# orybkin/video-gcp

Measured on AMD Instinct MI355X. Metric: predicted frames/sec, 64x64x3 seq_len=80 gcp_tree (posterior forward + all loss terms, model(inputs) and model.loss() of train.py:157-159, batch-stat BatchNorm), higher is better.
Workload: dtype f32 (encoder / decoder convs and the tree GEMMs from 512 rows: split-f16 MFMA with f32 accumulate, f32-equivalent; everything else exact f32 MFMA)

## Files before the change

include/gcpx.h:

```cpp
#ifndef GCPX_H
#define GCPX_H

#include <stdint.h>

#ifdef __cplusplus
extern "C" {
#endif

#define GCPX_VERSION 1

typedef enum gcpx_status {
    GCPX_OK = 0,
    GCPX_ERR_INVALID_ARG = -1,
    GCPX_ERR_UNSUPPORTED = -2,
    GCPX_ERR_HIP = -3,
    GCPX_ERR_COMM = -4
} gcpx_status;

typedef enum gcpx_act { GCPX_ACT_NONE = 0, GCPX_ACT_LRELU = 1, GCPX_ACT_TANH = 2 } gcpx_act;

int gcpx_version(void);
const char* gcpx_last_error(void);
int gcpx_conv_grid(void);

// ... 26 lines not shown
    int32_t Cout;
    int32_t out_pitch;
    int32_t upsample;
    int32_t out_act;
    int32_t head_mode;
    const float* wpk;
    const float* bias;
    float* out;
    float* images;
    float* stats_partial;
    const int32_t* raw_row_map;
    const int32_t* src_row_map;
    const int32_t* src_row_frames;
    int32_t n_src_rows;
    int32_t w_split_log2;
    const void* wpk_split;
    const int32_t* w_split_log2_dev;
    int32_t split_layout;
    int32_t nll_rows;
    const float* nll_target;
    float* nll_partial;
    const float* nll_row_weight;
    float nll_scale;
    int32_t _pad3;
    float* images_rows;
    int64_t images_rows_dup;
    const float* bwd_r;
    const float *bwd_scale, *bwd_shift, *bwd_mean, *bwd_rstd;
    const float* addend;
    int32_t addend_frame_div;
    int32_t _pad4;
} gcpx_conv_args;

typedef enum gcpx_split_layout { GCPX_SPLIT_PLAIN = 0, GCPX_SPLIT_ROWFOLD = 1, GCPX_SPLIT_HEAD32 = 2 } gcpx_split_layout;

int gcpx_conv3x3(const gcpx_conv_args* a, void* stream);
int gcpx_conv3x3_grid(const gcpx_conv_args* a);
int gcpx_conv4x4s2(const gcpx_conv_args* a, void* stream);
int gcpx_conv4x4s2_grid(void);
int gcpx_conv4x4s2_image(const float* x, const float* wpk, const float* bias, float* out,
                         int32_t F, int32_t Hin, int32_t Win, int32_t Cout, int32_t out_act, void* stream);

int gcpx_bn_finalize(const float* partial, int32_t n_partial, int32_t pitch, int32_t C, double count,
                     const float* gamma, const float* beta, float eps, float* scale, float* shift,
                     float* running_mean, float* running_var, float momentum, float* mean_out, float* rstd_out,
                     void* stream);
int gcpx_randn(float* out, int64_t n, uint64_t* state, void* stream);
int gcpx_bn_fold(const float* running_mean, const float* running_var, const float* gamma, const float* beta,
                 float eps, int32_t C, float* scale, float* shift, void* stream);

typedef struct gcpx_row_src {
    const float* ptr;
    const int32_t* rowidx;
    const float* scale;
    const float* shiftv;
    int64_t sb, sr;
    int32_t width;
    int32_t shift;
    int32_t act;
    int32_t cmod;
} gcpx_row_src;

typedef enum gcpx_gemm_epi {
    GCPX_EPI_NONE = 0,
    GCPX_EPI_LRELU = 1,
    GCPX_EPI_LSTM = 2,
    GCPX_EPI_GAUSS_SAMPLE = 3
// ... 500 lines not shown
```

video-gcp_amd/csrc/conv3x3_split.hip:

```cpp
#include "common.h"
#include "split_mfma.h"

#include <cstdlib>
#include <type_traits>

namespace {

struct SplitUpCfg {
    static constexpr int RW = 18, RH = 6, LW = 10, LH = 4, CC = 16, KS = 5;
    static constexpr int RAW_BYTES = LH * LW * CC * 4;
    static constexpr int PLANE_BYTES = RH * RW * 32;
    static constexpr int WAVE_BYTES = RAW_BYTES + 2 * PLANE_BYTES;
    static constexpr int NS = (LH * LW * 4 + 63) / 64;
    static constexpr int W_CHUNK_BYTES = KS * 2 * 1024;
    static int lds_bytes(int nchunk) { return nchunk * W_CHUNK_BYTES + 8 * WAVE_BYTES + 8 * 2 * 16 * 4; }
};

__global__ void __launch_bounds__(512, 2) conv3x3_up16_split_kernel(const gcpx_conv_args a, const int items_per_wave,
                                                                    const int nitems) {
    using Cfg = SplitUpCfg;
    constexpr int RW = Cfg::RW, RH = Cfg::RH, LW = Cfg::LW, LH = Cfg::LH, CC = Cfg::CC, NS = Cfg::NS, KS = Cfg::KS;
    extern __shared__ float4 smem4[];
    const int nchunk = a.Cin / CC;
    const char* wl = reinterpret_cast<const char*>(smem4);
    const int tid = threadIdx.x, lane = tid & 63;
    const int wave = __builtin_amdgcn_readfirstlane(tid >> 6);
    char* wbuf = reinterpret_cast<char*>(smem4) + nchunk * Cfg::W_CHUNK_BYTES + wave * Cfg::WAVE_BYTES;
    float* raw = reinterpret_cast<float*>(wbuf);
    char* hi = wbuf + Cfg::RAW_BYTES;
    float* red = reinterpret_cast<float*>(reinterpret_cast<char*>(smem4) + nchunk * Cfg::W_CHUNK_BYTES + 8 * Cfg::WAVE_BYTES);
    const int j = lane & 15, q = lane >> 4;
    const int H = a.Hout, W = a.Wout, Hin = a.Hin, Win = a.Win;
    const int ncb = W / 16, nrq = H / 4;

    for (int i = tid; i < nchunk * Cfg::W_CHUNK_BYTES / 16; i += 512) smem4[i] = reinterpret_cast<const float4*>(a.wpk_split)[i];
    __syncthreads();

// ... 1088 lines not shown
#pragma unroll
    for (int s = 1; s < 64; s <<= 1) m = fmaxf(m, __shfl_xor(m, s));
    if ((tid & 63) == 0) red[tid >> 6] = m;
    __syncthreads();
    m = red[0];
#pragma unroll
    for (int w = 1; w < 16; ++w) m = fmaxf(m, red[w]);
    int e = m > 0.f ? 14 + 127 - (int)((__float_as_uint(m) >> 23) & 0xff) : 0;
    e = max(-20, min(100, e));
    if (tid == 0) *log2_out = e;
    const float sc = __uint_as_float((unsigned)(127 + e) << 23);
    for (int i = tid; i < n; i += 1024) {
        const int k = idx[i];
        const float v = (k >= 0 ? theta[k] : 0.f) * sc;
        const _Float16 h1 = (_Float16)v;
        const _Float16 h2 = (_Float16)(v - (float)h1);
        const int o = (i >> 9) * 1024 + (i & 511);
        out[o] = h1;
        out[o + 512] = h2;
    }
}
}

extern "C" int gcpx_split_pack(const float* theta, const int32_t* idx, int32_t n, void* out, int32_t* log2_out, void* stream_) {
    GCPX_CHECK_ARG(theta && idx && out && log2_out, "null pointer");
    GCPX_CHECK_ARG(n > 0 && n % 512 == 0, "n must be a positive multiple of 512");
    hipLaunchKernelGGL(split_pack_kernel, dim3(1), dim3(1024), 0, reinterpret_cast<hipStream_t>(stream_), theta, idx, n,
                       reinterpret_cast<_Float16*>(out), log2_out);
    GCPX_CHECK_LAUNCH();
    return GCPX_OK;
}

int gcpx_launch_up32_split(const gcpx_conv_args* a, hipStream_t stream, int which, int grid) {
    if (which == 0) return launch_up32_split<2, 1>(a, stream, grid);
    if (which == 1) return launch_up32_split<2, 2>(a, stream, grid);
    return launch_up32_split<4, 2>(a, stream, grid);
}

int gcpx_launch_up16_fold(const gcpx_conv_args* a, hipStream_t stream, int grid) {
    using Cfg = FoldCfg;
    GCPX_CHECK_ARG(a->Cin == 32 && a->Cout == 16 && a->Hin % Cfg::R == 0 && a->Hout == 2 * a->Hin && a->Wout == 2 * a->Win && a->Wout % 16 == 0,
                   "row-folded block: 32 -> 16 channels, Hin a multiple of 4, output width a multiple of 16");
    GCPX_CHECK_ARG(a->src[0].C % 4 == 0 && (a->nsrc == 1 ? a->src[0].C == 32 : a->src[0].C + a->src[1].C == 32), "source channels");
    static const bool prio = getenv("GCPX_FOLD_NOPRIO") == nullptr;
    auto kern = prio ? conv3x3_up16_fold_kernel<true> : conv3x3_up16_fold_kernel<false>;
    static bool attr_set = false;
    if (!attr_set) {
        for (auto k : {conv3x3_up16_fold_kernel<true>, conv3x3_up16_fold_kernel<false>}) {
            hipError_t e = hipFuncSetAttribute(reinterpret_cast<const void*>(k), hipFuncAttributeMaxDynamicSharedMemorySize, Cfg::LDS_BYTES);
            if (e != hipSuccess) {
                gcpx_set_error("conv3x3 row-folded up16: hipFuncSetAttribute(%d B LDS): %s", Cfg::LDS_BYTES, hipGetErrorString(e));
                return GCPX_ERR_HIP;
            }
        }
        attr_set = true;
    }
    const int nitems = a->F * (a->Hin / Cfg::R) * (a->Wout / 16);
    const int ipw = (nitems + grid * 8 - 1) / (grid * 8);
    hipLaunchKernelGGL(kern, dim3(grid), dim3(512), Cfg::LDS_BYTES, stream, *a, ipw, nitems);
    GCPX_CHECK_LAUNCH();
    return GCPX_OK;
}

extern "C" int gcpx_fold_upsample_weights(const float* w, int32_t Cout, int32_t Cin, float* out, void* stream_) {
    GCPX_CHECK_ARG(w && out && Cout > 0 && Cin > 0, "bad arguments");
    const int n = 24 * Cout * Cin;
// ... 19 lines not shown
```

video-gcp_amd/forward_plan.py:

```python
import ctypes as C
import os
from contextlib import contextmanager

import torch

from . import packing as pk
from . import runtime as rt
from .hparams import GCPHParams
from .params import init_params, encoder_layers, encoder_skip_layers, decoder_layers
from .plan_ops import _Plan, _addr, N_LANES


class ForwardPlanMixin:

    def _plan_encoder(self, plan, tag, x_ptr, F, out_ptr, out_ob, out_orow, out_rpb):
        hp, P, lib = self._hp, self.pk, self.lib
        G = lib.gcpx_conv4x4s2_grid()
        S = hp.img_sz
        skip_idx = encoder_skip_layers(hp)
        skips = {}
        a0 = self._buf(f"{tag}.a0", (F, S // 2, S // 2, hp.ngf))
        enc_rec = dict(F=F, x_ptr=x_ptr, a0=a0, r={}, out=(out_ptr, out_ob, out_orow, out_rpb))
        plan.rec[f"enc:{tag}"] = enc_rec
        plan.add(f"enc.input:{tag}", lib.gcpx_conv4x4s2_image, x_ptr, P["enc.input.w"].data_ptr(),
# ... 37 lines not shown
        nrb = lib.gcpx_gemm_row_blocks(B * T, hp.nz_mid)
        st = self._buf(f"{tag}.st", (nrb, 2, hp.nz_mid)) if self.training else None
        self._gemm(plan, f"{tag}.pyramid-0", taps(y1, hp.nz_mid), B * T, hp.nz_mid, T, P[f"{tag}.pyramid-0.w"],
                   P[f"{tag}.pyramid-0.b"], out=y2.data_ptr(), ob=T * hp.nz_mid, orow=hp.nz_mid, stats=st)
        sc, sh = self._bn(plan, f"{tag}.bn", f"{prefix}.net.pyramid-0.norm", hp.nz_mid, st, nrb, hp.nz_mid, B * T)
        self._gemm(plan, f"{tag}.head", taps(y2, hp.nz_mid, scale=sc, shiftv=sh, act=rt.ACT_LRELU, cmod=hp.nz_mid),
                   B * T, nz, T, P[f"{tag}.head.w"], P[f"{tag}.head.b"], out=out.data_ptr(), ob=T * nz, orow=nz)

    def _plan_attention(self, plan, l, W, el, er, M, n, B, Kp, Vp, tin):
        hp, lib = self._hp, self.lib
        T, nz, dk = hp.max_seq_len, hp.nz_enc, hp.nz_attn_key
        li = l if hp.untied_layers else 0
        qin = self._buf(f"attn.qin{l}", (M, dk))
        self._mlp(plan, f"attn.query{l}", W["attn.query"], [el, er], M, n, out=qin.data_ptr(), ob=n * dk, orow=dk)
        dense = lambda t, w: self._rowsrc(t.data_ptr(), 0, w, w)
        qp = self._buf(f"attn.q{l}", (M, dk))
        self._gemm(plan, f"attn.q_proj{l}", [dense(qin, dk)], M, dk, M, W["attn.q_proj.w"], W["attn.q_proj.b"],
                   out=qp.data_ptr(), ob=0, orow=dk)
        o = self._buf(f"attn.o{l}", (M, nz))
        gamma = self._buf(f"attn.gamma{l}", (M, T))
        temp = self.sd[f"tree_module.tree_modules.{li}.inference.attention.attention_layers.0.temperature"]
        plan.add(f"attn{l}", lib.gcpx_attention, qp.data_ptr(), _addr(Kp, li * B * T * dk), _addr(Vp, li * B * T * nz), None,
                 tin["end_ind"].data_ptr(), temp.data_ptr(), o.data_ptr(), gamma.data_ptr(), M, n, T, dk, nz, hp.n_attention_heads)
        raw = self._buf(f"attn.raw{l}", (M, nz))
        self._gemm(plan, f"attn.out_proj{l}", [dense(o, nz)], M, nz, M, W["attn.out_proj.w"], W["attn.out_proj.b"],
                   out=raw.data_ptr(), ob=0, orow=nz)
        et = self._buf(f"attn.e_tilde{l}", (M, nz))
        self._gemm(plan, f"attn.out{l}", [dense(raw, nz)], M, nz, M, W["attn.out.w"], W["attn.out.b"], out=et.data_ptr(), ob=0, orow=nz)
        plan.rec.setdefault("gamma", {})[l] = gamma
        plan.rec.setdefault("e_tilde", {})[l] = et
        plan.rec.setdefault("attn", {})[l] = dict(qin=qin, qp=qp, o=o, raw=raw, gamma=gamma, et=et, M=M, n=n, li=li, temp=temp)
        return self._rowsrc(et.data_ptr(), n * nz, nz, nz)

    def _plan_decoder_features(self, plan, e_src, F, rpb, skips):
        hp, P, lib = self._hp, self.pk, self.lib
        ctop = self._c_top
        d0 = self._buf("dec.d0", (F, 4, 4, ctop))
        plan.rec["dec"] = dict(F=F, rpb=rpb, e_src=e_src, d0=d0, blocks=[], skips=skips)
        nrb = lib.gcpx_gemm_row_blocks(F, 16 * ctop)
        st = self._buf("dec.st0", (nrb, 2, 16 * ctop)) if self.training else None
        self._gemm(plan, "dec.input", [e_src], F, 16 * ctop, rpb, P["dec.input.w"], P["dec.input.b"], out=d0.data_ptr(),
                   ob=rpb * 16 * ctop, orow=16 * ctop, stats=st)
        sc, sh = self._bn(plan, "dec.bn0", "decoder.net.input.norm", ctop, st, nrb, 16 * ctop, F * 16)
        prev = (d0.data_ptr(), ctop, 1, sc, sh, rt.ACT_LRELU)
        res = 4
        for name, c_prev, c_skip, skip_idx, cout in decoder_layers(hp):
            srcs = [prev]
            if skip_idx >= 0:
                t, C_, ssc, ssh, sact = skips[skip_idx]
                assert C_ == c_skip and t.shape[1] == res
                srcs.append((t.data_ptr(), C_, rpb, ssc, ssh, sact))
            o = self._buf(f"dec.{name}", (F, 2 * res, 2 * res, cout))
            cpad = (cout + 15) // 16 * 16
            hoist = (skip_idx >= 0 and rpb > 1 and F % rpb == 0 and self.split_f16 and cout in (32, 64) and c_prev % 32 == 0 and
                     c_skip % 32 == 0 and f"dec.{name}" in self.pk_split and "fold" not in self.pk_split[f"dec.{name}"] and
                     os.environ.get("GCPX_NO_SKIP_HOIST") is None)
            addend = None
            if hoist:
                addend = self._buf(f"dec.{name}.skip", (F // rpb, 2 * res, 2 * res, cout))
                t, C_, ssc, ssh, sact = skips[skip_idx]
                zb = self._buf(f"dec.{name}.zero_bias", (cpad,), zero=True)
                a_s = self._conv_args([(t.data_ptr(), C_, 1, ssc, ssh, sact)], F // rpb, res, res, 2 * res, 2 * res, cout, cout,
                                      P[f"dec.{name}.w"], zb, addend, upsample=1)
                self._set_split(a_s, f"dec.{name}")
                a_s.wpk_split = a_s.wpk_split + (c_prev // 32) * 9 * (cpad // 16) * 2048
                plan.keep.append(a_s)
                plan.add(f"dec.{name}.skip", lib.gcpx_conv3x3, C.byref(a_s))
                srcs_main = [prev]
            else:
                srcs_main = srcs
            a = self._conv_args(srcs_main, F, res, res, 2 * res, 2 * res, cout, cout, P[f"dec.{name}.w"], P[f"dec.{name}.b"],
                                o, upsample=1, stats=(o if self.training else None))
            if hoist:
                a.addend, a.addend_frame_div = addend.data_ptr(), rpb
            self._set_split(a, f"dec.{name}")
            Gl = lib.gcpx_conv3x3_grid(C.byref(a))
            assert Gl > 0, rt.lib().gcpx_last_error()
            st = self._buf(f"dec.st.{name}", (Gl, 2, cpad)) if self.training else None
            a.stats_partial = st.data_ptr() if st is not None else None
            plan.keep.append(a)
            plan.add(f"dec.{name}", lib.gcpx_conv3x3, C.byref(a))
            plan.rec["dec"]["blocks"].append(dict(name=name, srcs=srcs, out=o, res_in=res, cout=cout, c_prev=c_prev, c_skip=c_skip,
                                                  skip_idx=skip_idx))
            res *= 2
            sc, sh = self._bn(plan, f"dec.bn.{name}", f"decoder.net.{name}.norm", cout, st, Gl, cpad, F * res * res)
            prev = (o.data_ptr(), cout, 1, sc, sh, rt.ACT_LRELU)
        assert res == hp.img_sz
        return prev

    def _build_plan(self, key, tin):
        hp, P, lib = self._hp, self.pk, self.lib
        B, has_traj, has_z, sample_prior, phase = key[0], key[1], key[2], key[3], key[4]
        pred_len = key[9]
        train_aux = has_traj and phase == "train" and not sample_prior
        L, T, N = hp.hierarchy_levels, hp.max_seq_len, hp.n_nodes
        nz, nv, H, SD = hp.nz_enc, hp.nz_vae, hp.nz_mid_lstm, hp.lstm_state_dim
        PS = 2 ** L + 1
        plan = _Plan(lib)
        G = lib.gcpx_conv_grid()
        def plan_aux_indices():
# ... 44 lines not shown
                if hp.seq_enc == "none":
                    inf_enc = enc_traj
                else:
                    inf_enc = self._buf("inf_enc_seq", (B * T, nz))
                    self._plan_seq_encoder(plan, "seq", "inf_encoder", enc_traj, inf_enc, B)
                if attentive:
                    dk = hp.nz_attn_key
                    n_mod = L if hp.untied_layers else 1
                    if hp.seq_enc == "none":
                        kenc = enc_traj
                    else:
                        kenc = self._buf("inf_key_enc", (B * T, nz))
                        self._plan_seq_encoder(plan, "kseq", "inf_key_encoder.0", enc_traj, kenc, B)
                    keys = self._buf("inf_enc_key_seq", (B * T, dk))
                    dense = lambda t, w: self._rowsrc(t.data_ptr(), 0, w, w)
                    self._gemm(plan, "kseq.key", [dense(kenc, nz)], B * T, dk, B * T, P["kseq.key.w"], P["kseq.key.b"],
                               out=keys.data_ptr(), ob=0, orow=dk)
                    Kp = self._buf("attn.K", (n_mod, B * T, dk))
                    Vp = self._buf("attn.V", (n_mod, B * T, nz))
                    self._gemm(plan, "attn.k_proj", [dense(keys, dk)], B * T, dk, B * T, P["attn.k_proj.w"], P["attn.k_proj.b"],
                               out=Kp.data_ptr(), ob=0, orow=dk, batch=(n_mod, 0, P["attn.k_proj.w"][0].numel(), dk, B * T * dk))
                    self._gemm(plan, "attn.v_proj", [dense(inf_enc, nz)], B * T, nz, B * T, P["attn.v_proj.w"], P["attn.v_proj.b"],
                               out=Vp.data_ptr(), ob=0, orow=nz, batch=(n_mod, 0, P["attn.v_proj.w"][0].numel(), nz, B * T * nz))
                    plan.rec["attn_kv"] = dict(Kp=Kp, Vp=Vp, keys=keys, kenc=kenc, n_mod=n_mod)

        if traj_first:
            plan_traj_encoder()
        plan.lane = 1
        if "rng_all" in tin:
            plan.add("randn", lib.gcpx_randn, tin["rng_all"].data_ptr(), tin["rng_all"].numel(), self._buf("rng_state", (2,), torch.int64).data_ptr())
            if "aux_n" in tin and not pred_len:
                plan.wait(2, 1)
        skips = self._plan_encoder(plan, "I0", tin["I_0"].data_ptr(), B, _addr(E), PS * nz, 0, 1)
        plan.lane = 2
        if not pred_len:
            if "aux_n" in tin:
                plan_aux_indices()
            plan_bookkeeping()
        if hp.attach_cost_mdl and hp.run_cost_mdl and train_aux and self._has_aux_training:
            gt = self._buf("cost_target", (B,))
            rows = hp.input_nc * hp.img_sz
            plan.add("path_cost", lib.gcpx_path_cost, tin["traj_seq"].data_ptr(), tin["cost_start_idx"].data_ptr(),
                     tin["cost_end_idx"].data_ptr(), B, T, rows, hp.img_sz, self._buf("cost_partial", (B, rows)).data_ptr(), gt.data_ptr())
        self._plan_encoder(plan, "Ig", tin["I_g"].data_ptr(), B, _addr(E, 2 ** L * nz), PS * nz, 0, 1)
        outs = {}
        e0 = lambda: self._rowsrc(_addr(E), PS * nz, 0, nz)
        eg = lambda: self._rowsrc(_addr(E, 2 ** L * nz), PS * nz, 0, nz)
        if hp.regress_length and not pred_len:
            plan.wait(2, 1)
            logits = self._buf("seq_len_logits", (B, T))
            self._mlp(plan, "length_pred", P["length_pred"], [e0(), eg()], B, 1, out=logits.data_ptr(), ob=T, orow=0)
            outs["seq_len_logits"] = logits
        if not traj_first:
            plan_traj_encoder()
        plan.lane = 0
        plan.join([1, 2])

        if hp.regress_length and pred_len:
            logits = self._buf("seq_len_logits", (B, T))
            self._mlp(plan, "length_pred", P["length_pred"], [e0(), eg()], B, 1, out=logits.data_ptr(), ob=T, orow=0)
            outs["seq_len_logits"] = logits
            plan.add("sample_length", lib.gcpx_sample_length, logits.data_ptr(), tin["len_u"].data_ptr(), B, T, 2, tin["end_ind"].data_ptr())
            plan_bookkeeping()

        side_merge = False
        for l in range(L):
# ... 351 lines not shown
```

video-gcp_amd/packing.py:

```python
import torch

_LANE = torch.arange(64)
_LI = _LANE % 16
_LQ = _LANE // 16


def _pad_rows(w, rows):
    if w.shape[0] == rows:
        return w
    pad = torch.zeros((rows - w.shape[0],) + tuple(w.shape[1:]), dtype=w.dtype, device=w.device)
    return torch.cat([w, pad], 0)


def pack_gemm(w):
    N, K = w.shape
    assert K % 16 == 0, (N, K)
    NT = (N + 15) // 16
    w = _pad_rows(w, NT * 16)
    dev = w.device
    kg = torch.arange(K // 16, device=dev)[:, None, None, None]
    nt = torch.arange(NT, device=dev)[None, :, None, None]
    li = _LI.to(dev)[None, None, :, None]
    lq = _LQ.to(dev)[None, None, :, None]
    s = torch.arange(4, device=dev)[None, None, None, :]
# ... 287 lines not shown
    out = []
    for py in range(2):
        for dyl in range(3):
            for tx in range(3):
                c = _FOLD_CF[py][dyl]
                s = c[0] * wd[:, :, 0, tx]
                s = s + c[1] * wd[:, :, 1, tx]
                s = s + c[2] * wd[:, :, 2, tx]
                out.append(s)
    out += [-wd[:, :, 0, tx] for tx in range(3)] + [-wd[:, :, 2, tx] for tx in range(3)]
    return torch.stack(out, 0).float()


def conv3x3_fold_gather(fw):
    assert fw.shape == (24, 16, 32)
    dev = fw.device
    t = torch.arange(24, device=dev)[:, None, None]
    li = _LI.to(dev)[None, :, None]
    lq = _LQ.to(dev)[None, :, None]
    el = torch.arange(8, device=dev)[None, None, :]
    return fw[t, li, lq * 8 + el].contiguous()


def pack_conv3x3_fold(w):
    w1, w2, e = split_f16(conv3x3_fold_gather(fold_up_weights(w)))
    return torch.stack([w1, w2], 1).contiguous().view(torch.int16), e


def conv3x3_fold_index():
    ids = torch.arange(24 * 16 * 32, dtype=torch.float64).view(24, 16, 32)
    return conv3x3_fold_gather(ids).reshape(-1).to(torch.int32)


def lstm_gate_interleave(w_ih, w_hh, b_ih, b_hh):
    H = w_hh.shape[1]
    w = torch.cat([w_ih, w_hh], dim=1)
    K = w.shape[1]
    w = w.view(4, H, K).permute(1, 0, 2).reshape(4 * H, K)
    b = (b_ih + b_hh).view(4, H).t().reshape(4 * H)
    return w.contiguous(), b.contiguous()
```

video-gcp_amd/runtime.py:

```python
import ctypes as C
import os

_HERE = os.path.dirname(os.path.abspath(__file__))
LIB_PATH = os.path.join(_HERE, "libgcpx.so")

ACT_NONE, ACT_LRELU, ACT_TANH = 0, 1, 2
HEAD_RAW, HEAD_DLM_MEAN, HEAD_DLM_BOTH, HEAD_TANH_NCHW, HEAD_DLM_NLL, HEAD_DLM_NLL_GRAD = 0, 1, 2, 3, 4, 5
SPLIT_PLAIN, SPLIT_ROWFOLD, SPLIT_HEAD32 = 0, 1, 2
EPI_NONE, EPI_LRELU, EPI_LSTM, EPI_GAUSS_SAMPLE = 0, 1, 2, 3
MLP_PLAIN, MLP_GAUSS, MLP_TANH = 0, 1, 2

vp = C.c_void_p
i32 = C.c_int32
i64 = C.c_int64


class ConvSrc(C.Structure):
    _fields_ = [("ptr", vp), ("scale", vp), ("shift", vp), ("C", i32), ("frame_div", i32), ("act", i32), ("_pad", i32)]


class ConvArgs(C.Structure):
    _fields_ = [("src", ConvSrc * 2), ("nsrc", i32), ("F", i32), ("Hin", i32), ("Win", i32), ("Hout", i32),
                ("Wout", i32), ("Cin", i32), ("Cout", i32), ("out_pitch", i32), ("upsample", i32), ("out_act", i32),
                ("head_mode", i32), ("wpk", vp), ("bias", vp), ("out", vp), ("images", vp), ("stats_partial", vp),
                ("raw_row_map", vp), ("src_row_map", vp), ("src_row_frames", vp), ("n_src_rows", i32), ("w_split_log2", i32), ("wpk_split", vp), ("w_split_log2_dev", vp),
                ("split_layout", i32), ("nll_rows", i32), ("nll_target", vp), ("nll_partial", vp), ("nll_row_weight", vp),
                ("nll_scale", C.c_float), ("_pad3", i32), ("images_rows", vp), ("images_rows_dup", i64), ("bwd_r", vp), ("bwd_scale", vp), ("bwd_shift", vp), ("bwd_mean", vp),
                ("bwd_rstd", vp), ("addend", vp), ("addend_frame_div", i32), ("_pad4", i32)]


class LossArgs(C.Structure):
    _fields_ = [("nll_bt", vp), ("pad_mask", vp), ("kl_b", vp), ("len_logits", vp), ("end_ind", vp), ("existence", vp),
                ("leave", vp), ("regressed_state", vp), ("state_target", vp), ("seq_len", vp), ("out", vp),
                ("B", i32), ("T", i32), ("N", i32), ("state_dim", i32), ("w_rec", C.c_float), ("w_kl", C.c_float),
                ("w_len", C.c_float), ("w_exist", C.c_float), ("w_state", C.c_float), ("total_div", C.c_float),
                ("action_pred", vp), ("action_seq", vp), ("inv_t0", vp), ("cost_pred", vp), ("cost_target", vp),
                ("n_actions", i32), ("w_action", C.c_float), ("w_cost", C.c_float), ("state_mask", vp), ("w_kl_dev", vp)]


class RowSrc(C.Structure):
    _fields_ = [("ptr", vp), ("rowidx", vp), ("scale", vp), ("shiftv", vp), ("sb", i64), ("sr", i64),
# ... 271 lines not shown
```

video-gcp_amd/weights.py:

```python
import ctypes as C
import os
from contextlib import contextmanager

import torch

from . import packing as pk
from . import runtime as rt
from .hparams import GCPHParams
from .params import init_params, encoder_layers, encoder_skip_layers, decoder_layers
from .plan_ops import _addr


class WeightsMixin:

    def _flatten_params(self, params):
        off, self._poff = 0, {}
        for k, v in params.items():
            self._poff[k] = (off, tuple(v.shape))
            off += (v.numel() + 3) // 4 * 4
        self.theta = torch.zeros(off, dtype=torch.float32, device=self.device)
        self.sd = {}
        for k, v in params.items():
            o, shp = self._poff[k]
            view = self.theta[o:o + v.numel()].view(shp)
            view.copy_(v)
            self.sd[k] = view

    def _pack_predictor(self, prefix, out_dim):
        sd = self._psd
        mid = sd[f"{prefix}.input.linear.weight"].shape[0]
        n_mid = 0
        while f"{prefix}.pyramid-{n_mid}.linear.weight" in sd:
            n_mid += 1
        out_pad = (out_dim + 15) // 16 * 16
        w_in = sd[f"{prefix}.input.linear.weight"]
        k_raw = w_in.shape[1]
        if k_raw % 16:
            w_in = torch.cat([w_in, torch.zeros((mid, -k_raw % 16), dtype=w_in.dtype, device=w_in.device)], 1)
        d = dict(mid=mid, n_mid=n_mid, out_dim=out_dim, in_dim=w_in.shape[1], in_dim_raw=k_raw)
        d["w_in"] = pk.pack_gemm(w_in)
        d["b_in"] = sd[f"{prefix}.input.linear.bias"].contiguous()
        if n_mid:
            d["w_mid"] = torch.stack([pk.pack_gemm(sd[f"{prefix}.pyramid-{i}.linear.weight"]) for i in range(n_mid)]).contiguous()
            d["b_mid"] = torch.stack([sd[f"{prefix}.pyramid-{i}.linear.bias"] for i in range(n_mid)]).contiguous()
            d["gn_g"] = torch.stack([sd[f"{prefix}.pyramid-{i}.norm.weight"] for i in range(n_mid)]).contiguous()
            d["gn_b"] = torch.stack([sd[f"{prefix}.pyramid-{i}.norm.bias"] for i in range(n_mid)]).contiguous()
        d["w_out"] = pk.pack_gemm(sd[f"{prefix}.head.linear.weight"])
        d["b_out"] = pk.pad_vec(sd[f"{prefix}.head.linear.bias"], out_pad)
        return d

    def _pack_all(self):
        if self._arena is not None:
            self.repack()
            return
        self.pk = self._pack_tree(self.sd)
        if self._hp.tree_lstm:
            self._pack_fused_embed()
        self._pack_split()
        self._pack_gemm_split()

    def _pack_split(self):
        self.pk_split = {}
        hp = self._hp
        todo = []
        if hp.decoder_distribution == "discrete_logistic_mixture":
            todo.append(("dec.head", "decoder.gen_head.conv.weight", pk.dlm_channel_perm(hp.n_mixtures)))
            if self.head32 and hp.n_mixtures == 10 and hp.head_channels == 100:
                todo.append(("dec.head32", "decoder.gen_head.conv.weight", ("head32", pk.dlm_channel_perm(hp.n_mixtures))))
        for name, c_prev, c_skip, skip_idx, cout in decoder_layers(hp):
            if cout == 16 and c_prev + c_skip == 32:
                todo.append((f"dec.{name}", f"decoder.net.{name}.conv.weight", "rowfold"))
            elif cout == 16:
                todo.append((f"dec.{name}", f"decoder.net.{name}.conv.weight", None))
            elif cout in (32, 64) and (c_prev + c_skip) % 32 == 0:
                todo.append((f"dec.{name}", f"decoder.net.{name}.conv.weight", "tiled32"))
        for name, cin, cout, norm in self._enc_layers[1:]:
            if cin == 16 or cin % 32 == 0:
                todo.append((f"enc.{name}", f"encoder.net.{name}.conv.weight", "enc4x4"))
        for name, key, perm in todo:
            off, shp = self._poff[key]
            d = {}
            if perm == "enc4x4":
                idx = pk.conv4x4_split_index(shp, off).to(self.device)
            elif perm == "rowfold":
                d["fold"] = torch.zeros(24 * shp[0] * shp[1], dtype=torch.float32, device=self.device)
                d["fold_src"] = (off, shp[0], shp[1])
                idx = pk.conv3x3_fold_index().to(self.device)
            elif perm == "tiled32":
                idx = pk.conv3x3_split32_index(shp, off).to(self.device)
            elif isinstance(perm, tuple) and perm[0] == "head32":
                idx = pk.head32_index(shp, off, perm[1]).to(self.device)
            else:
                idx = pk.conv3x3_split_index(shp, off, perm).to(self.device)
            d.update(idx=idx, out=torch.zeros(2 * idx.numel(), dtype=torch.int16, device=self.device),
                     log2=torch.zeros(1, dtype=torch.int32, device=self.device))
            self.pk_split[name] = d
        self.repack_split()

    def repack_split(self, stream=None):
        st = stream if stream is not None else torch.cuda.current_stream(self.device).cuda_stream
        if not self.pk_split:
            return
        tab = self._split_tab
        key = (self.theta.data_ptr(),) + tuple((d["out"].data_ptr(), d["idx"].data_ptr()) for d in self.pk_split.values())
        if tab is None or tab[2] != key:
            descs = []
            for name, d in self.pk_split.items():
                src = d["fold"] if "fold" in d else self.theta
                e = rt.SplitPackDesc()
                e.src, e.idx, e.out, e.log2_out, e.n = src.data_ptr(), d["idx"].data_ptr(), d["out"].data_ptr(), d["log2"].data_ptr(), d["idx"].numel()
                descs.append(e)
            arr = (rt.SplitPackDesc * len(descs))(*descs)
            dev = torch.frombuffer(bytearray(bytes(arr)), dtype=torch.uint8).to(self.device)
            tab = self._split_tab = (dev, len(descs), key, torch.zeros(len(descs), dtype=torch.int32, device=self.device))
        for name, d in self.pk_split.items():
            if "fold_src" in d:
                off, cout, cin = d["fold_src"]
                rt.check(self.lib.gcpx_fold_upsample_weights(self.theta.data_ptr() + 4 * off, cout, cin, d["fold"].data_ptr(), st), "fold_upsample_weights")
        rt.check(self.lib.gcpx_split_pack_group2(tab[0].data_ptr(), tab[1], tab[3].data_ptr(), st), "split_pack_group2")

    def _pack_gemm_split(self):
        self._gsplit = {}
        self._merge_side_rows = int(os.environ.get("GCPX_MERGE_SIDE_ROWS", "512")) or (1 << 60)
        pr = int(os.environ.get("GCPX_GEMM_PLANES_ROWS", "512"))
        self._planes_min_rows = pr if pr > 0 else 1 << 60
        if not self.split_f16:
            return
        for name, W in self.pk.items():
            if not (isinstance(W, dict) and name.startswith("tree")):
                continue
            for key, wpk in W.items():
                if not (key.endswith(".w") and (key.startswith("lstm") or key == "proj.w")):
                    continue
                stack = wpk if wpk.dim() == 5 else wpk[None]
                if (stack.shape[2] * 16) % 64 or (stack.shape[1] * 16) % 64:
                    continue
                packs = [pk.pack_gemm_split(pk.unpack_gemm(w, w.shape[1] * 16)) for w in stack]
                ws = torch.stack([p_[0] for p_ in packs]).contiguous().to(self.device)
                es = torch.tensor([p_[1] for p_ in packs], dtype=torch.int32, device=self.device)
                self._gsplit[wpk.data_ptr()] = (ws, es)

    def _set_split(self, a, name):
        d = self.pk_split.get(name)
        layout = None
        if name == "dec.head" and self.head32 and a.head_mode in (rt.HEAD_DLM_MEAN, rt.HEAD_DLM_NLL, rt.HEAD_DLM_NLL_GRAD) \
                and "dec.head32" in self.pk_split:
            d, layout = self.pk_split["dec.head32"], rt.SPLIT_HEAD32
        if self.split_f16 and d is not None:
            a.wpk_split, a.w_split_log2_dev = d["out"].data_ptr(), d["log2"].data_ptr()
            if layout is None:
                layout = rt.SPLIT_ROWFOLD if "fold" in d else rt.SPLIT_PLAIN
            a.split_layout = layout

    def _pack_fused_embed(self):
        hp = self._hp
        for l in range(hp.hierarchy_levels if hp.untied_layers else 1):
            p = f"tree_module.tree_modules.{l}.subgoal_pred"
            sd = self.sd
            We, be = sd[f"{p}.embed.weight"].double(), sd[f"{p}.embed.bias"].double()
            Wih = sd[f"{p}.lstm.0.weight_ih"].double()
            Wf = (Wih @ We).float()
            bf = (Wih @ be).float() + sd[f"{p}.lstm.0.bias_ih"]
            w, b = pk.lstm_gate_interleave(Wf, sd[f"{p}.lstm.0.weight_hh"], bf, sd[f"{p}.lstm.0.bias_hh"])
            self.pk[f"tree{l}"]["lstm0f.w"], self.pk[f"tree{l}"]["lstm0f.b"] = pk.pack_gemm(w), b

    def _pack_tree(self, sd):
        hp = self._hp
        self._psd = sd
        P = {}
        layers, c_top = encoder_layers(hp)
        self._enc_layers, self._c_top = layers, c_top
        P["enc.input.w"] = pk.pack_conv4x4_image(sd["encoder.net.input.conv.weight"])
        P["enc.input.b"] = sd["encoder.net.input.conv.bias"].contiguous()
        for name, cin, cout, norm in layers[1:]:
            P[f"enc.{name}.w"] = pk.pack_conv4x4(sd[f"encoder.net.{name}.conv.weight"])
            P[f"enc.{name}.b"] = sd[f"encoder.net.{name}.conv.bias"].contiguous()
        wh = sd["encoder.net.head.weight"]
        P["enc.head.w"] = pk.pack_gemm(wh.permute(0, 2, 3, 1).reshape(hp.nz_enc, 16 * c_top))
        P["enc.head.b"] = sd["encoder.net.head.bias"].contiguous()
        wt = sd["decoder.net.input.conv.weight"]
        P["dec.input.w"] = pk.pack_gemm(wt.permute(2, 3, 1, 0).reshape(16 * c_top, hp.nz_enc))
        P["dec.input.b"] = sd["decoder.net.input.conv.bias"].repeat(16).contiguous()
        for name, c_prev, c_skip, skip_idx, cout in decoder_layers(hp):
            P[f"dec.{name}.w"] = pk.pack_conv3x3(sd[f"decoder.net.{name}.conv.weight"], 16 if cout == 16 else 32)
# ... 199 lines not shown
```

Measured before the change: 501,800.

## Add row-folded up32 split conv and plan skip-half convs right after the I0 encoder

```diff
diff --git a/include/gcpx.h b/include/gcpx.h
--- a/include/gcpx.h
+++ b/include/gcpx.h
@@ -82,7 +82,7 @@
     int32_t _pad4;
 } gcpx_conv_args;
 
-typedef enum gcpx_split_layout { GCPX_SPLIT_PLAIN = 0, GCPX_SPLIT_ROWFOLD = 1, GCPX_SPLIT_HEAD32 = 2 } gcpx_split_layout;
+typedef enum gcpx_split_layout { GCPX_SPLIT_PLAIN = 0, GCPX_SPLIT_ROWFOLD = 1, GCPX_SPLIT_HEAD32 = 2, GCPX_SPLIT_ROWFOLD32 = 3 } gcpx_split_layout;
 
 int gcpx_conv3x3(const gcpx_conv_args* a, void* stream);
 int gcpx_conv3x3_grid(const gcpx_conv_args* a);
diff --git a/video-gcp_amd/csrc/conv3x3_split.hip b/video-gcp_amd/csrc/conv3x3_split.hip
--- a/video-gcp_amd/csrc/conv3x3_split.hip
+++ b/video-gcp_amd/csrc/conv3x3_split.hip
@@ -3,6 +3,8 @@
 
 #include <cstdlib>
 #include <type_traits>
+
+int gcpx_launch_up32_fold(const gcpx_conv_args* a, hipStream_t stream, int which, int grid);
 
 namespace {
 
@@ -1157,6 +1159,7 @@
 }
 
 int gcpx_launch_up32_split(const gcpx_conv_args* a, hipStream_t stream, int which, int grid) {
+    if (a->split_layout == GCPX_SPLIT_ROWFOLD32) return gcpx_launch_up32_fold(a, stream, which, grid);
     if (which == 0) return launch_up32_split<2, 1>(a, stream, grid);
     if (which == 1) return launch_up32_split<2, 2>(a, stream, grid);
     return launch_up32_split<4, 2>(a, stream, grid);
diff --git a/video-gcp_amd/csrc/conv3x3_up32_fold.hip b/video-gcp_amd/csrc/conv3x3_up32_fold.hip
--- /dev/null
+++ b/video-gcp_amd/csrc/conv3x3_up32_fold.hip
@@ -0,0 +1,342 @@
+#include "split_common.h"
+
+namespace {
+
+template <int TILE> struct FoldTileShape;
+template <> struct FoldTileShape<1> { static constexpr int TH = 16, TW = 16, TF = 1; };
+template <> struct FoldTileShape<2> { static constexpr int TH = 8, TW = 8, TF = 4; };
+
+template <int CT, int TILE>
+struct Fold32Cfg {
+    using TS = FoldTileShape<TILE>;
+    static constexpr int TH = TS::TH, TW = TS::TW, TF = TS::TF, CC = 32, C4 = 8;
+    static constexpr int LH = TH / 2 + 2, LW = TW / 2 + 2, RW = TW + 2;
+    static constexpr int FRAME_BYTES = LH * RW * 64 + (TF > 1 ? 128 : 0);
+    static constexpr int PLANE_BYTES = TF * FRAME_BYTES;
+    static constexpr int RAW_BYTES = TF * LH * LW * CC * 4;
+    static constexpr int LDS_BYTES = 2 * PLANE_BYTES + RAW_BYTES + 64;
+    static constexpr int NSLOT = TF * LH * LW * C4;
+    static constexpr int NS = (NSLOT + 255) / 256;
+    static constexpr int NOUT = TF * LH * RW * C4;
+    static constexpr int NO = (NOUT + 255) / 256;
+    static constexpr int DEPTH = 2, NSET = DEPTH + 1;
+    static constexpr int CH = CT / 2, NG = 12 * CH;
+    static constexpr int STEP_BYTES = CT * 2048;
+};
+
+template <int CT, int TILE>
+__global__ void __launch_bounds__(256, 2) conv3x3_up32_fold_kernel(const gcpx_conv_args a, const int ntx, const int nty, const int ntiles) {
+    using Cfg = Fold32Cfg<CT, TILE>;
+    constexpr int TH = Cfg::TH, TW = Cfg::TW, TF = Cfg::TF, LH = Cfg::LH, LW = Cfg::LW, RW = Cfg::RW;
+    constexpr int CC = Cfg::CC, C4 = Cfg::C4, NS = Cfg::NS, NSLOT = Cfg::NSLOT, NO = Cfg::NO, NOUT = Cfg::NOUT;
+    constexpr int CH = Cfg::CH, NG = Cfg::NG, DEPTH = Cfg::DEPTH, NSET = Cfg::NSET, SB = Cfg::STEP_BYTES, PR = 4;
+    static_assert(CT % 2 == 0 && NG % NSET == 0, "the weight register sets rotate through a chunk's granules");
+    extern __shared__ float4 smem4[];
+    char* hi = reinterpret_cast<char*>(smem4);
+    float* raw = reinterpret_cast<float*>(hi + 2 * Cfg::PLANE_BYTES);
+    float* wmax = reinterpret_cast<float*>(hi + 2 * Cfg::PLANE_BYTES + Cfg::RAW_BYTES);
+
+    const int tid = threadIdx.x;
+    const int lane = tid & 63, wave = __builtin_amdgcn_readfirstlane(tid >> 6);
+    const int j = lane & 15, q = lane >> 4;
+    const int nchunk = a.Cin / CC;
+    const int Hout = a.Hout, Wout = a.Wout, F = a.F;
+    const int ew = a.w_split_log2_dev ? __builtin_amdgcn_readfirstlane(*a.w_split_log2_dev) : a.w_split_log2;
+
+    const int py = wave & 1, g = wave >> 1;
+    const int yl0 = (TILE == 1) ? 4 * g : 0;
+    const int pfl = (TILE == 1) ? 0 : 2 * g + (j >> 3);
+    const int px = (TILE == 1) ? j : (j & 7);
+    const int bbase = pfl * Cfg::FRAME_BYTES + (yl0 * RW + px) * 64 + q * 16;
+
+    auto slot = [&](int k, int& c4, int& rx, int& ry, int& fl, int& lds) {
+        const int idx = tid + 256 * k;
+        c4 = idx % C4;
+        int t = idx / C4;
+        rx = t % LW; t /= LW;
+        ry = t % LH;
+        fl = (idx < NSLOT) ? t / LH : -1;
+        lds = ((fl * LH + ry) * LW + rx) * CC + c4 * 4;
+    };
+    const char* wbase = reinterpret_cast<const char*>(a.wpk_split) + lane * 16;
+    const char* wpar = wbase + py * 9 * SB;
+    const char* wbord = wbase + (18 + 3 * py) * SB;
+    const int brow = py ? 5 * RW * 64 : 0;
+
+    f32x4 st1[CT], st2[CT];
+#pragma unroll
+    for (int ct = 0; ct < CT; ++ct) { st1[ct] = f32x4{0, 0, 0, 0}; st2[ct] = f32x4{0, 0, 0, 0}; }
+
+    float4 pre[NS];
+    unsigned pre_ok = 0;
+    auto tile_origin = [&](int tile, int& f0, int& y0, int& x0) {
+        const int tx = tile % ntx;
+        const int t2 = tile / ntx;
+        f0 = (t2 / nty) * TF; y0 = (t2 % nty) * TH; x0 = tx * TW;
+    };
+    auto issue_loads = [&](int tile, int chunk) {
+        int f0, y0, x0;
+        tile_origin(tile, f0, y0, x0);
+        pre_ok = 0;
+        const int c0 = a.src[0].C;
+#pragma unroll
+        for (int k = 0; k < NS; ++k) {
+            pre[k] = make_float4(0.f, 0.f, 0.f, 0.f);
+            int s_c4, s_rx, s_ry, s_fl, s_lds;
+            slot(k, s_c4, s_rx, s_ry, s_fl, s_lds);
+            if (s_fl < 0) continue;
+            const int f = f0 + s_fl;
+            if (f < F) {
+                const int sy = min(max(y0 / 2 - 1 + s_ry, 0), a.Hin - 1);
+                const int sx = min(max(x0 / 2 - 1 + s_rx, 0), a.Win - 1);
+                const int cg = chunk * CC + s_c4 * 4;
+                const bool first = cg < c0;
+                const gcpx_conv_src& sr = first ? a.src[0] : a.src[1];
+                const int cl = first ? cg : cg - c0;
+                pre[k] = *reinterpret_cast<const float4*>(sr.ptr + (((size_t)(f / sr.frame_div) * a.Hin + sy) * a.Win + sx) * sr.C + cl);
+                pre_ok |= 1u << k;
+            }
+        }
+    };
+    auto wload = [&](const int chunk_, const int gi, h8 (&w)[2][2]) __attribute__((always_inline)) {
+        const int s = gi / CH, h = gi % CH;
+        const char* wp0 = s < 9 ? wpar + ((s % 3) * 3 + s / 3) * SB : wbord + (s - 9) * SB;
+        const char* wp = wp0 + (size_t)min(chunk_, nchunk - 1) * 24 * SB + h * 4096;
+#pragma unroll
+        for (int c = 0; c < 2; ++c) {
+            w[c][0] = *reinterpret_cast<const h8*>(wp + c * 2048);
+            w[c][1] = *reinterpret_cast<const h8*>(wp + c * 2048 + 1024);
+        }
+    };
+    auto load_b = [&](const int tx, const int r, h8 (&b)[2]) __attribute__((always_inline)) {
+        const char* bp = hi + bbase + (r * RW + tx) * 64;
+        b[0] = *reinterpret_cast<const h8*>(bp);
+        b[1] = *reinterpret_cast<const h8*>(bp + Cfg::PLANE_BYTES);
+    };
+
+    int tile = blockIdx.x;
+    if (tile < ntiles) issue_loads(tile, 0);
+    for (; tile < ntiles; tile += gridDim.x) {
+        int f0, y0, x0;
+        tile_origin(tile, f0, y0, x0);
+        f32x4 acc[CT][PR];
+#pragma unroll
+        for (int ct = 0; ct < CT; ++ct)
+#pragma unroll
+            for (int pt = 0; pt < PR; ++pt) acc[ct][pt] = f32x4{0, 0, 0, 0};
+        int ex = 0;
+        const bool top = (y0 == 0), bot = (y0 + TH == Hout), lft = (x0 == 0), rgt = (x0 + TW == Wout);
+        const bool has_b = (py == 0) ? (top && (TILE != 1 || g == 0)) : (bot && (TILE != 1 || g == 1));
+
+        h8 wr[NSET][2][2];
+#pragma unroll
+        for (int k = 0; k < DEPTH; ++k) wload(0, k, wr[k]);
+
+#pragma unroll 1
+        for (int chunk = 0; chunk < nchunk; ++chunk) {
+            float amax = 0.f;
+            {
+                const int c0 = a.src[0].C;
+#pragma unroll
+                for (int k = 0; k < NS; ++k) {
+                    int s_c4, s_rx, s_ry, s_fl, s_lds;
+                    slot(k, s_c4, s_rx, s_ry, s_fl, s_lds);
+                    if (s_fl < 0) continue;
+                    float4 v = pre[k];
+                    if (pre_ok & (1u << k)) {
+                        const int cg = chunk * CC + s_c4 * 4;
+                        const bool first = cg < c0;
+                        const gcpx_conv_src& sr = first ? a.src[0] : a.src[1];
+                        v = affine_act4(v, sr.scale, sr.shift, first ? cg : cg - c0, sr.act);
+                    }
+                    *reinterpret_cast<float4*>(raw + s_lds) = v;
+                    amax = fmaxf(amax, fmaxf(fmaxf(fabsf(v.x), fabsf(v.y)), fmaxf(fabsf(v.z), fabsf(v.w))));
+                }
+            }
+#pragma unroll
+            for (int m = 1; m < 64; m <<= 1) amax = fmaxf(amax, __shfl_xor(amax, m));
+            if (lane == 0) wmax[wave] = amax;
+            __syncthreads();
+            amax = fmaxf(fmaxf(wmax[0], wmax[1]), fmaxf(wmax[2], wmax[3]));
+            int ec = 14 + 127 - (int)((__float_as_uint(amax) >> 23) & 0xff);
+            ec = __builtin_amdgcn_readfirstlane(amax > 0.f ? max(-100, min(min(100, 126 - ew), ec)) : min(100, 126 - ew));
+            if (chunk == 0) ex = ec;
+            else if (ec < ex) {
+                const float r = __uint_as_float((unsigned)(127 + ec - ex) << 23);
+#pragma unroll
+                for (int ct = 0; ct < CT; ++ct)
+#pragma unroll
+                    for (int pt = 0; pt < PR; ++pt) acc[ct][pt] *= r;
+                ex = ec;
+            }
+            const float sx2 = __uint_as_float((unsigned)__builtin_amdgcn_readfirstlane((127 + ex) << 23));
+#pragma unroll
+            for (int k = 0; k < NO; ++k) {
+                const int idx = tid + 256 * k;
+                if (NOUT % 256 != 0 && k == NO - 1 && idx >= NOUT) break;
+                const int c4 = idx & (C4 - 1);
+                const int p = idx >> 3;
+                const int cx = p % RW, t = p / RW;
+                const float* rp = raw + (t * LW + (cx >> 1)) * CC + c4 * 4;
+                const float4 A = *reinterpret_cast<const float4*>(rp);
+                const float4 B = *reinterpret_cast<const float4*>(rp + CC);
+                const bool zero = (lft && cx == 0) || (rgt && cx == RW - 1);
+                const float wa = zero ? 0.f : ((cx & 1) ? 0.25f : 0.75f);
+                const float wb = zero ? 0.f : ((cx & 1) ? 0.75f : 0.25f);
+                float4 v;
+                v.x = fmaf(wa, A.x, wb * B.x); v.y = fmaf(wa, A.y, wb * B.y); v.z = fmaf(wa, A.z, wb * B.z); v.w = fmaf(wa, A.w, wb * B.w);
+                h4 p1, p2;
+                split4(v, sx2, p1, p2);
+                char* dst = hi + idx * 8 + (t / LH) * (Cfg::FRAME_BYTES - LH * RW * 64);
+                *reinterpret_cast<h4*>(dst) = p1;
+                *reinterpret_cast<h4*>(dst + Cfg::PLANE_BYTES) = p2;
+            }
+            __syncthreads();
+            if (chunk + 1 < nchunk) issue_loads(tile, chunk + 1);
+            else if (tile + (int)gridDim.x < ntiles) issue_loads(tile + gridDim.x, 0);
+
+            h8 bq[2][6][2];
+#pragma unroll
+            for (int r = 0; r < 4; ++r) load_b(0, r, bq[0][r]);
+            __builtin_amdgcn_s_setprio(1);
+            h8 bb[3][2];
+            static_for<0, NG>([&](auto gc_) __attribute__((always_inline)) {
+                constexpr int gi = decltype(gc_)::value, s = gi / CH, h = gi % CH;
+                constexpr int gn = gi + DEPTH;
+                if constexpr (gn < NG) wload(chunk, gn, wr[gn % NSET]);
+                else wload(chunk + 1, gn - NG, wr[gn % NSET]);
+                const auto& wc = wr[gi % NSET];
+                if constexpr (s < 9) {
+                    constexpr int tx = s / 3, dyl = s % 3;
+                    if constexpr (h == 0) {
+                        if constexpr (dyl == 0) {
+                            load_b(tx, 4, bq[tx & 1][4]);
+                            load_b(tx, 5, bq[tx & 1][5]);
+                        } else if constexpr (tx + 1 < 3) {
+                            load_b(tx + 1, 2 * (dyl - 1), bq[(tx + 1) & 1][2 * (dyl - 1)]);
+                            load_b(tx + 1, 2 * (dyl - 1) + 1, bq[(tx + 1) & 1][2 * (dyl - 1) + 1]);
+                        }
+                    }
+                    if constexpr (gi == 9 * CH - 1) {
+#pragma unroll
+                        for (int t = 0; t < 3; ++t) {
+                            const char* bp = hi + bbase + brow + t * 64;
+                            bb[t][0] = *reinterpret_cast<const h8*>(bp);
+                            bb[t][1] = *reinterpret_cast<const h8*>(bp + Cfg::PLANE_BYTES);
+                        }
+                    }
+#pragma unroll
+                    for (int c = 0; c < 2; ++c) {
+#pragma unroll
+                        for (int pt = 0; pt < PR; ++pt) acc[2 * h + c][pt] = mfma32h(wc[c][1], bq[tx & 1][pt + dyl][0], acc[2 * h + c][pt]);
+#pragma unroll
+                        for (int pt = 0; pt < PR; ++pt) acc[2 * h + c][pt] = mfma32h(wc[c][0], bq[tx & 1][pt + dyl][1], acc[2 * h + c][pt]);
+#pragma unroll
+                        for (int pt = 0; pt < PR; ++pt) acc[2 * h + c][pt] = mfma32h(wc[c][0], bq[tx & 1][pt + dyl][0], acc[2 * h + c][pt]);
+                    }
+                } else {
+                    constexpr int tx = s - 9;
+                    if (has_b && py == 0) {
+#pragma unroll
+                        for (int c = 0; c < 2; ++c) {
+                            acc[2 * h + c][0] = mfma32h(wc[c][1], bb[tx][0], acc[2 * h + c][0]);
+                            acc[2 * h + c][0] = mfma32h(wc[c][0], bb[tx][1], acc[2 * h + c][0]);
+                            acc[2 * h + c][0] = mfma32h(wc[c][0], bb[tx][0], acc[2 * h + c][0]);
+                        }
+                    } else if (has_b) {
+#pragma unroll
+                        for (int c = 0; c < 2; ++c) {
+                            acc[2 * h + c][3] = mfma32h(wc[c][1], bb[tx][0], acc[2 * h + c][3]);
+                            acc[2 * h + c][3] = mfma32h(wc[c][0], bb[tx][1], acc[2 * h + c][3]);
+                            acc[2 * h + c][3] = mfma32h(wc[c][0], bb[tx][0], acc[2 * h + c][3]);
+                        }
+                    }
+                }
+            });
+            __builtin_amdgcn_s_setprio(0);
+        }
+
+        const float inv = __uint_as_float((unsigned)(127 - ex - ew) << 23);
+        const int f = f0 + pfl;
+        if (f < F) {
+#pragma unroll
+            for (int pt = 0; pt < PR; ++pt) {
+                const int oy = y0 + 2 * (yl0 + pt) + py, ox = x0 + px;
+                float* op = a.out + (((size_t)f * Hout + oy) * Wout + ox) * a.out_pitch;
+#pragma unroll
+                for (int ct = 0; ct < CT; ++ct) {
+                    const float4 bv = *reinterpret_cast<const float4*>(a.bias + ct * 16 + q * 4);
+                    f32x4 v = acc[ct][pt];
+                    v[0] = fmaf(v[0], inv, bv.x); v[1] = fmaf(v[1], inv, bv.y); v[2] = fmaf(v[2], inv, bv.z); v[3] = fmaf(v[3], inv, bv.w);
+                    if (a.addend) {
+                        const float4 ad = *reinterpret_cast<const float4*>(a.addend + (((size_t)(f / a.addend_frame_div) * Hout + oy) * Wout + ox) *
+                                                                                          a.out_pitch + ct * 16 + q * 4);
+                        v[0] += ad.x; v[1] += ad.y; v[2] += ad.z; v[3] += ad.w;
+                    }
+                    *reinterpret_cast<float4*>(op + ct * 16 + q * 4) = make_float4(v[0], v[1], v[2], v[3]);
+                    if (a.stats_partial) {
+                        st1[ct] += v;
+                        st2[ct] += v * v;
+                    }
+                }
+            }
+        }
+    }
+
+    if (a.stats_partial) {
+        __syncthreads();
+        float* red = reinterpret_cast<float*>(hi);
+#pragma unroll
+        for (int ct = 0; ct < CT; ++ct) {
+#pragma unroll
+            for (int r = 0; r < 4; ++r) {
+                const float s1 = row16_sum(st1[ct][r]);
+                const float s2 = row16_sum(st2[ct][r]);
+                if (j == 0) {
+                    red[(wave * 2 + 0) * CT * 16 + ct * 16 + q * 4 + r] = s1;
+                    red[(wave * 2 + 1) * CT * 16 + ct * 16 + q * 4 + r] = s2;
+                }
+            }
+        }
+        __syncthreads();
+        if (tid < 2 * CT * 16) {
+            const int which = tid / (CT * 16), c = tid % (CT * 16);
+            float sum = 0.f;
+#pragma unroll
+            for (int w = 0; w < 4; ++w) sum += red[(w * 2 + which) * CT * 16 + c];
+            a.stats_partial[((size_t)blockIdx.x * 2 + which) * CT * 16 + c] = sum;
+        }
+    }
+}
+
+template <int CT, int TILE>
+int launch_up32_fold(const gcpx_conv_args* a, hipStream_t stream, int grid) {
+    using Cfg = Fold32Cfg<CT, TILE>;
+    const int ntx = a->Wout / Cfg::TW, nty = a->Hout / Cfg::TH;
+    const int nfg = (a->F + Cfg::TF - 1) / Cfg::TF;
+    auto kern = conv3x3_up32_fold_kernel<CT, TILE>;
+    static bool attr_set = false;
+    if (!attr_set) {
+        hipError_t e = hipFuncSetAttribute(reinterpret_cast<const void*>(kern), hipFuncAttributeMaxDynamicSharedMemorySize, Cfg::LDS_BYTES);
+        if (e != hipSuccess) {
+            gcpx_set_error("conv3x3 row-folded up32: hipFuncSetAttribute(%d B LDS): %s", Cfg::LDS_BYTES, hipGetErrorString(e));
+            return GCPX_ERR_HIP;
+        }
+        attr_set = true;
+    }
+    hipLaunchKernelGGL(kern, dim3(grid), dim3(256), Cfg::LDS_BYTES, stream, *a, ntx, nty, ntx * nty * nfg);
+    GCPX_CHECK_LAUNCH();
+    return GCPX_OK;
+}
+
+}
+
+int gcpx_launch_up32_fold(const gcpx_conv_args* a, hipStream_t stream, int which, int grid) {
+    const int TW = which == 0 ? 16 : 8, CT = which == 2 ? 4 : 2;
+    GCPX_CHECK_ARG(a->upsample && a->Hout == 2 * a->Hin && a->Wout == 2 * a->Win && a->Wout % TW == 0 && a->Hout % TW == 0,
+                   "row-folded block: bilinear x2, output a multiple of the tile");
+    GCPX_CHECK_ARG(a->Cin % 32 == 0 && a->Cout == CT * 16 && a->src[0].C % 4 == 0, "row-folded block: Cin a multiple of 32, 32 / 64 output channels");
+    if (which == 0) return launch_up32_fold<2, 1>(a, stream, grid);
+    if (which == 1) return launch_up32_fold<2, 2>(a, stream, grid);
+    return launch_up32_fold<4, 2>(a, stream, grid);
+}
diff --git a/video-gcp_amd/forward_plan.py b/video-gcp_amd/forward_plan.py
--- a/video-gcp_amd/forward_plan.py
+++ b/video-gcp_amd/forward_plan.py
@@ -93,6 +93,25 @@
         plan.rec.setdefault("attn", {})[l] = dict(qin=qin, qp=qp, o=o, raw=raw, gamma=gamma, et=et, M=M, n=n, li=li, temp=temp)
         return self._rowsrc(et.data_ptr(), n * nz, nz, nz)
 
+    def _skip_hoistable(self, name, c_prev, c_skip, cout):
+        d = self.pk_split.get(f"dec.{name}")
+        return bool(self.split_f16 and cout in (32, 64) and c_prev % 32 == 0 and c_skip % 32 == 0 and d is not None and
+                    ("fold" not in d or "fold32" in d) and os.environ.get("GCPX_NO_SKIP_HOIST") is None)
+
+    def _plan_skip_half(self, plan, name, c_prev, cout, res, skip, nseq):
+        t, C_, ssc, ssh, sact = skip
+        cpad = (cout + 15) // 16 * 16
+        addend = self._buf(f"dec.{name}.skip", (nseq, 2 * res, 2 * res, cout))
+        zb = self._buf(f"dec.{name}.zero_bias", (cpad,), zero=True)
+        a_s = self._conv_args([(t.data_ptr(), C_, 1, ssc, ssh, sact)], nseq, res, res, 2 * res, 2 * res, cout, cout,
+                              self.pk[f"dec.{name}.w"], zb, addend, upsample=1)
+        self._set_split(a_s, f"dec.{name}")
+        nset = 24 if "fold32" in self.pk_split[f"dec.{name}"] else 9
+        a_s.wpk_split = a_s.wpk_split + (c_prev // 32) * nset * (cpad // 16) * 2048
+        plan.keep.append(a_s)
+        plan.add(f"dec.{name}.skip", self.lib.gcpx_conv3x3, C.byref(a_s))
+        return addend
+
     def _plan_decoder_features(self, plan, e_src, F, rpb, skips):
         hp, P, lib = self._hp, self.pk, self.lib
         ctop = self._c_top
@@ -113,20 +132,12 @@
                 srcs.append((t.data_ptr(), C_, rpb, ssc, ssh, sact))
             o = self._buf(f"dec.{name}", (F, 2 * res, 2 * res, cout))
             cpad = (cout + 15) // 16 * 16
-            hoist = (skip_idx >= 0 and rpb > 1 and F % rpb == 0 and self.split_f16 and cout in (32, 64) and c_prev % 32 == 0 and
-                     c_skip % 32 == 0 and f"dec.{name}" in self.pk_split and "fold" not in self.pk_split[f"dec.{name}"] and
-                     os.environ.get("GCPX_NO_SKIP_HOIST") is None)
+            hoist = skip_idx >= 0 and rpb > 1 and F % rpb == 0 and self._skip_hoistable(name, c_prev, c_skip, cout)
             addend = None
             if hoist:
-                addend = self._buf(f"dec.{name}.skip", (F // rpb, 2 * res, 2 * res, cout))
-                t, C_, ssc, ssh, sact = skips[skip_idx]
-                zb = self._buf(f"dec.{name}.zero_bias", (cpad,), zero=True)
-                a_s = self._conv_args([(t.data_ptr(), C_, 1, ssc, ssh, sact)], F // rpb, res, res, 2 * res, 2 * res, cout, cout,
-                                      P[f"dec.{name}.w"], zb, addend, upsample=1)
-                self._set_split(a_s, f"dec.{name}")
-                a_s.wpk_split = a_s.wpk_split + (c_prev // 32) * 9 * (cpad // 16) * 2048
-                plan.keep.append(a_s)
-                plan.add(f"dec.{name}.skip", lib.gcpx_conv3x3, C.byref(a_s))
+                addend = plan.rec.get("dec_skip_addend", {}).get((name, F // rpb))
+                if addend is None:
+                    addend = self._plan_skip_half(plan, name, c_prev, cout, res, skips[skip_idx], F // rpb)
                 srcs_main = [prev]
             else:
                 srcs_main = srcs
@@ -237,6 +248,12 @@
             if "aux_n" in tin and not pred_len:
                 plan.wait(2, 1)
         skips = self._plan_encoder(plan, "I0", tin["I_0"].data_ptr(), B, _addr(E), PS * nz, 0, 1)
+        if key[8] and N > 1 and os.environ.get("GCPX_SKIP_INLINE") is None:
+            res_ = 4
+            for name, c_prev, c_skip, skip_idx, cout in decoder_layers(hp):
+                if skip_idx >= 0 and self._skip_hoistable(name, c_prev, c_skip, cout):
+                    plan.rec.setdefault("dec_skip_addend", {})[(name, B)] = self._plan_skip_half(plan, name, c_prev, cout, res_, skips[skip_idx], B)
+                res_ *= 2
         plan.lane = 2
         if not pred_len:
             if "aux_n" in tin:
diff --git a/video-gcp_amd/packing.py b/video-gcp_amd/packing.py
--- a/video-gcp_amd/packing.py
+++ b/video-gcp_amd/packing.py
@@ -343,6 +343,30 @@
     return conv3x3_fold_gather(ids).reshape(-1).to(torch.int32)
 
 
+def conv3x3_fold32_gather(fw):
+    T, Cout, Cin = fw.shape
+    assert T == 24 and Cin % 32 == 0 and Cout % 16 == 0
+    dev = fw.device
+    ch = torch.arange(Cin // 32, device=dev)[:, None, None, None, None]
+    t = torch.arange(24, device=dev)[None, :, None, None, None]
+    ct = torch.arange(Cout // 16, device=dev)[None, None, :, None, None]
+    li = _LI.to(dev)[None, None, None, :, None]
+    lq = _LQ.to(dev)[None, None, None, :, None]
+    el = torch.arange(8, device=dev)[None, None, None, None, :]
+    return fw[t, ct * 16 + li, ch * 32 + lq * 8 + el].contiguous()
+
+
+def pack_conv3x3_fold32(w):
+    w1, w2, e = split_f16(conv3x3_fold32_gather(fold_up_weights(w)))
+    return torch.stack([w1, w2], 3).contiguous().view(torch.int16), e
+
+
+def conv3x3_fold32_index(shape):
+    cout, cin = shape[0], shape[1]
+    ids = torch.arange(24 * cout * cin, dtype=torch.float64).view(24, cout, cin)
+    return conv3x3_fold32_gather(ids).reshape(-1).to(torch.int32)
+
+
 def lstm_gate_interleave(w_ih, w_hh, b_ih, b_hh):
     H = w_hh.shape[1]
     w = torch.cat([w_ih, w_hh], dim=1)
diff --git a/video-gcp_amd/runtime.py b/video-gcp_amd/runtime.py
--- a/video-gcp_amd/runtime.py
+++ b/video-gcp_amd/runtime.py
@@ -6,7 +6,7 @@
 
 ACT_NONE, ACT_LRELU, ACT_TANH = 0, 1, 2
 HEAD_RAW, HEAD_DLM_MEAN, HEAD_DLM_BOTH, HEAD_TANH_NCHW, HEAD_DLM_NLL, HEAD_DLM_NLL_GRAD = 0, 1, 2, 3, 4, 5
-SPLIT_PLAIN, SPLIT_ROWFOLD, SPLIT_HEAD32 = 0, 1, 2
+SPLIT_PLAIN, SPLIT_ROWFOLD, SPLIT_HEAD32, SPLIT_ROWFOLD32 = 0, 1, 2, 3
 EPI_NONE, EPI_LRELU, EPI_LSTM, EPI_GAUSS_SAMPLE = 0, 1, 2, 3
 MLP_PLAIN, MLP_GAUSS, MLP_TANH = 0, 1, 2
 
diff --git a/video-gcp_amd/weights.py b/video-gcp_amd/weights.py
--- a/video-gcp_amd/weights.py
+++ b/video-gcp_amd/weights.py
@@ -9,6 +9,8 @@
 from .hparams import GCPHParams
 from .params import init_params, encoder_layers, encoder_skip_layers, decoder_layers
 from .plan_ops import _addr
+
+ROWFOLD32_COUT = ()
 
 
 class WeightsMixin:
@@ -73,7 +75,9 @@
             elif cout == 16:
                 todo.append((f"dec.{name}", f"decoder.net.{name}.conv.weight", None))
             elif cout in (32, 64) and (c_prev + c_skip) % 32 == 0:
-                todo.append((f"dec.{name}", f"decoder.net.{name}.conv.weight", "tiled32"))
+                on_ = os.environ.get("GCPX_ROWFOLD32", "")
+                fold = cout in ROWFOLD32_COUT or on_ == "1" or str(cout) in on_.split(",")
+                todo.append((f"dec.{name}", f"decoder.net.{name}.conv.weight", "rowfold32" if fold else "tiled32"))
         for name, cin, cout, norm in self._enc_layers[1:]:
             if cin == 16 or cin % 32 == 0:
                 todo.append((f"enc.{name}", f"encoder.net.{name}.conv.weight", "enc4x4"))
@@ -86,6 +90,11 @@
                 d["fold"] = torch.zeros(24 * shp[0] * shp[1], dtype=torch.float32, device=self.device)
                 d["fold_src"] = (off, shp[0], shp[1])
                 idx = pk.conv3x3_fold_index().to(self.device)
+            elif perm == "rowfold32":
+                d["fold"] = torch.zeros(24 * shp[0] * shp[1], dtype=torch.float32, device=self.device)
+                d["fold_src"] = (off, shp[0], shp[1])
+                d["fold32"] = True
+                idx = pk.conv3x3_fold32_index(shp).to(self.device)
             elif perm == "tiled32":
                 idx = pk.conv3x3_split32_index(shp, off).to(self.device)
             elif isinstance(perm, tuple) and perm[0] == "head32":
@@ -149,7 +158,7 @@
         if self.split_f16 and d is not None:
             a.wpk_split, a.w_split_log2_dev = d["out"].data_ptr(), d["log2"].data_ptr()
             if layout is None:
-                layout = rt.SPLIT_ROWFOLD if "fold" in d else rt.SPLIT_PLAIN
+                layout = rt.SPLIT_ROWFOLD32 if "fold32" in d else rt.SPLIT_ROWFOLD if "fold" in d else rt.SPLIT_PLAIN
             a.split_layout = layout
 
     def _pack_fused_embed(self):
```

Result: no change. 504,900, median of 6 (+0.6%).
